# mckerrigan/shadow

Measured on AMD Instinct MI355X. Metric: source-paths/sec, higher is better.
Workload: dtype f64; 1 GPU; c4_as50k: Barabasi-Albert Internet-like topology, all-pairs latency/reliability table (BASELINE.json configs[3]); n_vertices=50000, n_edges=550000, n_edges_nonloop=500000, csr_arcs=1000000, targets=50000, table_bytes=40000000000, parallelism=one GPU

## Files before the change

### shadow_amd/csrc/engine.hip

```cpp
#include "common.hpp"

#include <array>
#include <atomic>
#include <chrono>
#include <condition_variable>
#include <functional>
#include <map>
#include <memory>
#include <mutex>
#include <sys/mman.h>

#include <thread>
#include "sssp_f64.hpp"
#include "sssp_f64d.hpp"
#include "sssp_k32.hpp"
#include "sssp_batch.hpp"
#include "path_attr.hpp"
#include "sssp_delta.hpp"
#include "direct_fw.hpp"
#include "fw.hpp"
#include "path_hops.hpp"
#include "link_loads.hpp"
#include "path_ties.hpp"
#include "ecmp_loads.hpp"
// ... 235 lines not shown
        if (rc) return rc;
        if (s.kf.h) {
            if (hipMalloc((void**)&c->d_kf_ws, s.kf.ws_stride * (size_t)s.kf.slots) != hipSuccess) return SHD_ROUTE_ENOMEM;
            c->allocs.push_back(c->d_kf_ws);
        }
    }
    c->h_ridx = std::move(s.kd.oridx);
    s.arrays([](const char*, auto& h, auto*&) { std::remove_reference_t<decltype(h)>().swap(h); });
    s.inrows.order = {}; s.inrows.src_of = {};
    c->sel = s.sel;
    c->inrows = std::move(s.inrows); c->k32 = std::move(s.k32); c->attr = s.attr;
    c->kb = std::move(s.kb); c->kd = std::move(s.kd); c->kf = std::move(s.kf);
    return SHD_ROUTE_OK;
}

DevDelta kd_args(const shd_route* c) {
    DevDelta k;
    k.n = c->n; k.nw = (c->n + 63) / 64; k.bound = c->k32.bound; k.delta = c->kd.delta;
    k.fused = c->kd.fused; k.rc = c->kd.qcap;
    k.row = c->d_row; k.orec = c->kd.d_orec; k.oridx = c->kd.d_oridx;
    k.nnz = c->nnz; k.lrow = c->kd.d_lrow; k.lrec = reinterpret_cast<const uint2*>(c->kd.d_lrec); k.nlight = c->kd.nlight;
    k.rtab = c->kd.d_rtab; k.nrtab = c->kd.nrtab; k.rone = c->kd.rone; k.walk = c->kd.walk; k.packed = c->kd.packed;
    k.vf = c->d_vf; k.self_w = c->d_self_w; k.self_r = c->d_self_r; k.dbg = c->d_dbg; k.dflags = 0;
    k.has_vf = c->vf_lossy;
#ifdef SHD_STAMPS
    if (const char* e = getenv("SHD_ROUTE_DFLAGS")) k.dflags = atoi(e);
#endif
    k.seed_drop = 0;
    if (const char* e = getenv("SHD_ROUTE_SEEDDROP")) k.seed_drop = atoi(e) & ~1;

    k.jobs = nullptr; k.drow = nullptr; k.drow_out = nullptr; k.prow = nullptr; k.rstride = 0; k.evcap = c->n;
    k.done = nullptr;
    if (const char* e = getenv("SHD_ROUTE_EVCAP")) k.evcap = std::max(0, std::min(c->n, atoi(e)));
    k.next = nullptr;
    k.stats = c->d_kd_stats;
    return k;
}

int kd_launch(shd_route* c, DevDelta k, int* next, const int32_t* d_src, int ns, const int32_t* d_tgt, int nt,
              int64_t ld, double* d_lat, double* d_rel, double* d_row_min, hipStream_t st, bool planner = false,
              char* ws = nullptr, int max_grid = 0, bool hub = false) {
    if (ns <= 0) return SHD_ROUTE_OK;
    k.next = next;
    if (!ws) ws = c->d_kd_ws;
    const int grid = std::min(ns, max_grid > 0 ? std::min(max_grid, c->kd.slots) : c->kd.slots);
    const bool big = hub && planner && c->kd.hub_block > 0;
    size_t lds = c->kd.lds;
    if (big) { k.rc = c->kd.hub_qcap; k.delta = c->kd.hub_delta; lds = c->kd.hub_lds; }
    kd_dispatch(big ? c->kd.hub_block : c->kd.block, [&](auto B) {
        constexpr int b = decltype(B)::value;
        if (planner)
            hipLaunchKernelGGL(kd_plan_rows_kernel<b>, dim3(grid), dim3(b), lds, st, k, d_src, ns, d_tgt,
                               nt, (long long)ld, d_lat, d_rel, d_row_min, c->d_err, ws, c->kd.stride);
        else
            hipLaunchKernelGGL(sssp_delta_kernel<b>, dim3(grid), dim3(b), c->kd.lds, st, k, d_src, ns, d_tgt,
                               nt, (long long)ld, d_lat, d_rel, d_row_min, c->d_err, ws, c->kd.stride);
        return 0;
    });
    return hip_check(hipGetLastError());
}

DevKB kb_args(const shd_route* c, int ns) {
    DevKB kb;
    kb.n = c->n; kb.nnz = c->nnz; kb.nseg = c->kb.nseg; kb.nhub = c->kb.nhub; kb.npart = c->kb.npart;
    kb.bound = c->k32.bound; kb.arc = c->kb.fused ? c->kb.d_farc : c->kb.d_arc; kb.row_in = c->inrows.d_irow;
    kb.seg = c->kb.d_seg; kb.hub = c->kb.d_hub;
// ... 1000 lines not shown
```

### shadow_amd/csrc/sssp_delta.hpp

```cpp
#pragma once
#include "common.hpp"

namespace shd {

constexpr int KD_P = 8;
static_assert(KD_P == 8, "owner markers are read as one u64 per lane");
constexpr int KD_TAIL = 4;
constexpr int KD_W = 8;
constexpr int KD_IMP = 192;
constexpr uint32_t KD_NONE = 0xFFFFFFFFu;
constexpr uint32_t KD_SRC_MARK = 0xFFFFFFFEu;

#define KD_GLOBAL __attribute__((address_space(1)))

#ifndef KD_NSEEDS
#define KD_NSEEDS 3
#endif
constexpr int KD_SEEDS = KD_NSEEDS;
#ifndef KD_NTLOAD
#define KD_NTLOAD 1
#endif
#ifndef KD_JUMPS
#define KD_JUMPS 1
#endif
struct __attribute__((aligned(64))) KDJob {
    int row;
    int s;
    int store;
    int nseed;
    int seed[KD_SEEDS];
    int u[KD_SEEDS];
    int wr[KD_SEEDS];
    int rec[KD_SEEDS];
};
static_assert(sizeof(KDJob) == 64, "one 64-byte job record");
constexpr uint32_t KD_EVTAG = 0xFFFF0000u;
typedef unsigned short kd_us2 __attribute__((ext_vector_type(2)));
typedef double kd_d2 __attribute__((ext_vector_type(2)));
typedef unsigned kd_u4 __attribute__((ext_vector_type(4)));
typedef unsigned kd_u2 __attribute__((ext_vector_type(2)));

struct DevDelta {
    int* next;
    const KDJob* __restrict__ jobs;
    const uint16_t* __restrict__ drow;
    uint16_t* drow_out;
    uint32_t* prow;
    long long rstride;
    int evcap;
    int* done;
    int n, nw;
    int nlight;
    int nnz;
    int bound;
    int delta;
    int fused;
    int rc;
    const int* __restrict__ row;
    const uint32_t* __restrict__ orec;
    const uint16_t* __restrict__ oridx;
    const int* __restrict__ lrow;
    const uint2* __restrict__ lrec;
    const double* __restrict__ rtab;
    int nrtab;
    int rone;
    int walk;
    int packed;
    const double* __restrict__ vf;
    const double* __restrict__ self_w;
    const double* __restrict__ self_r;
    int has_vf;
    int dflags;
    int seed_drop;
    unsigned long long* dbg;
    unsigned long long* stats;
};

constexpr int KD_NACC = 40;
#ifdef SHD_STAMPS
#define KD_ACCP (sm->acc)
#define KD_OUT (!(dflags & 1))
#define KD_DFLAGS g.dflags
// ... 99 lines not shown
        L.ring = o;
        L.rrec = o + a16(2 * (size_t)rc);
        L.qcap = (int)((wbytes - 16) / 6) & ~7;
        L.qv = o;
        L.qbeg = o + a16(2 * (size_t)L.qcap);
        o += wbytes;
        L.total = o;
        L.rtabl = a16(L.rix + (size_t)n);
        return L;
    }
};
constexpr int KD_MAXD = 32;
#ifndef KD_SDIV
#define KD_SDIV 8
#endif
#ifndef KD_SMIN
#define KD_SMIN 16
#endif
#ifndef KD_WDYN
#define KD_WDYN 1
#endif
#ifndef KD_WCAP
#define KD_WCAP 2
#endif
#ifndef KD_SEEDSPIN
#define KD_SEEDSPIN 8
#endif
#ifndef KD_BWAVES
#define KD_BWAVES 8
#endif
#ifndef KD_BHELP
#define KD_BHELP 1
#endif
#ifndef KD_WQ_N
#define KD_WQ_N 2
#endif
constexpr int KD_WQ = KD_WQ_N;
constexpr int KD_ONE = 254;
constexpr int KD_NAN = 255;
constexpr int KD_RR = 512;
template <int B>
constexpr int kd_rr() { return B >= 1024 ? KD_RR : 256; }

__host__ __device__ inline size_t kd_ws_stride(int n) {
    return a16(sizeof(double) * n) + a16(sizeof(uint32_t) * (n + 8)) + a16(8 * (size_t)n) + 256 +
           a16(sizeof(uint32_t) * (n + 8));
}
__host__ __device__ inline size_t kd_ws_wpr1(int n) {
    return a16(sizeof(double) * n) + a16(sizeof(uint32_t) * (n + 8)) + a16(8 * (size_t)n) + 256;
}
__host__ __device__ inline long long kd_row_stride(int n) { return ((long long)n + 2 + 7) & ~7ll; }

__device__ inline void lds_barrier() { asm volatile("s_waitcnt lgkmcnt(0)\n\ts_barrier" ::: "memory"); }
__device__ inline void wait_stores() { asm volatile("s_waitcnt vmcnt(0)" ::: "memory"); }

__device__ inline unsigned kd_wave_min(unsigned x) {
#pragma unroll
    for (int d = 32; d >= 1; d >>= 1) x = min(x, (unsigned)__shfl_xor((int)x, d, 64));
    return x;
}

__device__ inline unsigned kd_wave_min_dpp(unsigned x) {
    int v = (int)x;
    const int inf = (int)0xFFFFFFFFu;
    v = (int)min((unsigned)v, (unsigned)__builtin_amdgcn_update_dpp(inf, v, 0x111, 0xF, 0xF, false));
    v = (int)min((unsigned)v, (unsigned)__builtin_amdgcn_update_dpp(inf, v, 0x112, 0xF, 0xF, false));
// ... 37 lines not shown
        "ds_bpermute_b32 %5, %18, %25\n\t"
        "ds_bpermute_b32 %6, %19, %24\n\t"
        "ds_bpermute_b32 %7, %19, %25\n\t"
        "ds_bpermute_b32 %8, %20, %24\n\t"
        "ds_bpermute_b32 %9, %20, %25\n\t"
        "ds_bpermute_b32 %10, %21, %24\n\t"
        "ds_bpermute_b32 %11, %21, %25\n\t"
        "ds_bpermute_b32 %12, %22, %24\n\t"
        "ds_bpermute_b32 %13, %22, %25\n\t"
        "ds_bpermute_b32 %14, %23, %24\n\t"
        "ds_bpermute_b32 %15, %23, %25\n\t"
        "s_waitcnt lgkmcnt(0)"
        : "=&v"(ob[0]), "=&v"(od[0]), "=&v"(ob[1]), "=&v"(od[1]), "=&v"(ob[2]), "=&v"(od[2]),
          "=&v"(ob[3]), "=&v"(od[3]), "=&v"(ob[4]), "=&v"(od[4]), "=&v"(ob[5]), "=&v"(od[5]),
          "=&v"(ob[6]), "=&v"(od[6]), "=&v"(ob[7]), "=&v"(od[7])
        : "v"(a[0]), "v"(a[1]), "v"(a[2]), "v"(a[3]), "v"(a[4]), "v"(a[5]), "v"(a[6]), "v"(a[7]),
          "v"(x), "v"(y));
}

__device__ inline unsigned ld16(const uint16_t* d, int v) { return d[v]; }
__device__ inline uint32_t kd_comp(const uint4& v, int k) { return k == 0 ? v.x : k == 1 ? v.y : k == 2 ? v.z : v.w; }

__device__ inline void pop4(unsigned long long* b, int k, int v[4]) {
#pragma unroll
    for (int q = 0; q < 4; q++) {
        const unsigned long long x = *b;
        v[q] = x ? (k << 6) + __ffsll((long long)x) - 1 : -1;
        *b = x & (x - 1);
    }
}

__device__ inline void kd_relax_list(const uint32_t* wimp, int cnt, int lane, unsigned long long upto,
                                     uint32_t* dist32, unsigned long long* pend, unsigned* wmin, uint16_t* ring,
                                     int* tail, int rc, unsigned T, unsigned long long* sm_acc) {
    __builtin_amdgcn_wave_barrier();
    for (int b0 = 0; b0 < cnt; b0 += 64) {
        const bool act = b0 + lane < cnt;
        const uint32_t e = act ? wimp[b0 + lane] : 0u;
        const unsigned v = e & 0xFFFFu, nd = e >> 16, sh = (v & 1u) << 4;
        bool won = false;
        if (act) {
            uint32_t old = dist32[v >> 1];
            for (;;) {
                if (nd >= ((old >> sh) & 0xFFFFu)) break;
                const uint32_t got = atomicCAS(&dist32[v >> 1], old, (old & ~(0xFFFFu << sh)) | (nd << sh));
                if (got == old) { won = true; break; }
                old = got;
            }
        }
        const bool push = won && nd < T;
        if (won && nd >= T) { atomicOr(&pend[v >> 6], 1ull << (v & 63)); atomicMin(&wmin[v >> 6], nd); }
        const unsigned long long pm = __ballot(push);
        if (pm) {
            const int ctot = __popcll(pm);
            int qb = 0;
            if (lane == 0) qb = atomicAdd(tail, ctot);
            qb = __builtin_amdgcn_readfirstlane(qb);
            const int qk = max(0, min(ctot, rc - qb));
            const int rk = __popcll(pm & (upto >> 1));
            if (push && rk < qk) { ring[qb + rk] = (uint16_t)v; atomicAnd(&pend[v >> 6], ~(1ull << (v & 63))); }
            if (push && rk >= qk) { atomicOr(&pend[v >> 6], 1ull << (v & 63)); atomicMin(&wmin[v >> 6], nd); }
#ifdef SHD_STAMPS
            if (lane == 0 && ctot > qk) atomicAdd(&sm_acc[14], (unsigned long long)(ctot - qk));
#endif
        }
    }
    __builtin_amdgcn_wave_barrier();
}


#define SEED_VIEW()                                                                                   \
    const int nseed = __builtin_amdgcn_readfirstlane(sm->job.nseed);                                   \
    int su[KD_SEEDS], sslot[KD_SEEDS];                                                                 \
    unsigned wsu[KD_SEEDS], rsu[KD_SEEDS];                                                             \
    const uint16_t* sdrow[KD_SEEDS];                                                                   \
    const uint32_t* sprow[KD_SEEDS];                                                                   \
    _Pragma("unroll") for (int q_ = 0; q_ < KD_SEEDS; q_++) {                                          \
        const int sl_ = __builtin_amdgcn_readfirstlane(q_ < nseed ? sm->job.seed[q_] : 0);             \
        const unsigned wr_ = (unsigned)__builtin_amdgcn_readfirstlane(q_ < nseed ? sm->job.wr[q_] : 0); \
        su[q_] = __builtin_amdgcn_readfirstlane(q_ < nseed ? sm->job.u[q_] : -1);                      \
        sslot[q_] = sl_; wsu[q_] = wr_ & 0xFFFFu;                                                      \
        rsu[q_] = (unsigned)__builtin_amdgcn_readfirstlane(q_ < nseed ? sm->job.rec[q_] : 0);          \
        sdrow[q_] = g.drow + (size_t)sl_ * g.rstride;                                                  \
        sprow[q_] = g.prow + (size_t)sl_ * g.rstride;                                                  \
    }                                                                                                  \
    (void)sslot; (void)rsu; (void)sprow; (void)su

__device__ inline int kd_next_source(int* ctr, int* slot, int tid, bool all_queued = false) {
    if (tid == 0) *slot = (all_queued ? 0 : (int)gridDim.x) + atomicAdd(ctr, 1);
    __syncthreads();
    const int i = *slot;
    __syncthreads();
    return i;
}

template <class T>
__device__ __attribute__((always_inline)) inline T kd_uni(T x) {
    if constexpr (sizeof(T) == 8) {
        unsigned long long b;
// ... 747 lines not shown
                const int r1 = e0 + (int)(e1 >> 16);
                const unsigned dv = ld16(dist, v);
                uint32_t fr = KD_NONE;
                bool open = have && a0 < r1;
                while (__ballot(open)) {
                    const int a = a0 + sub;
                    const kd_u2 ra = __builtin_amdgcn_raw_buffer_load_b64(ars, (uint32_t)a << 3, 0, 0);
                    const kd_u2 rb = __builtin_amdgcn_raw_buffer_load_b64(ars, (uint32_t)a << 3, 64, 0);
                    const unsigned da = ld16(dist, (int)(ra.x & 0xFFFFu)), db = ld16(dist, (int)(rb.x & 0xFFFFu));
                    const bool ta = open && a < r1 && da + (ra.x >> 16) == dv;
                    const bool tb = open && a + 8 < r1 && db + (rb.x >> 16) == dv;
                    const unsigned ma = (unsigned)(__ballot(ta) >> (8 * gi)) & 0xFFu;
                    const unsigned mb = (unsigned)(__ballot(tb) >> (8 * gi)) & 0xFFu;
                    const uint32_t ca = (ra.x & 0xFFFFu) | (ra.y << 16) | (packed ? (ra.x >> 16) << 24 : 0u);
                    const uint32_t cb = (rb.x & 0xFFFFu) | (rb.y << 16) | (packed ? (rb.x >> 16) << 24 : 0u);
                    const unsigned mm = ma ? ma : mb;
                    const int from = 8 * gi + (mm ? __ffs((int)mm) - 1 : 0);
                    const uint32_t got = (uint32_t)__shfl((int)(ma ? ca : cb), from, 64);
                    if (open && mm) { fr = got; open = false; }
                    if (open) { a0 += 16; open = a0 < r1; }
                }
                if (sub == 0 && have) {
                    if (fr == KD_NONE) raise_err(err, SHD_ROUTE_EUNREACH);
                    wpr[v] = fr;
                }
            }
            KD_WACC(17);
        }
        wait_stores();
        KD_WACC(16);
    }
}

#define KD_KERNEL_PARAMS                                                                              \
    DevDelta g, const int* __restrict__ src, int ns, const int* __restrict__ tgt, int nt, long long ld,     \
        double* __restrict__ lat_out, double* __restrict__ rel_out, double* __restrict__ row_min,          \
        int* __restrict__ err, char* __restrict__ ws, size_t ws_stride
template <int B>
__device__ __attribute__((always_inline)) inline void kd_rows_body(KD_KERNEL_PARAMS) {
    extern __shared__ __attribute__((aligned(16))) char smem[];
    const int n = g.n, nw = g.nw;
    constexpr int RR = kd_rr<B>();
    const KDLayout<B> L = KDLayout<B>::make(n, g.rc, RR);
    KDSmall* sm = reinterpret_cast<KDSmall*>(smem);
    const int tid = threadIdx.x, lane = tid & 63, wid = tid >> 6;
    uint32_t* wkey = reinterpret_cast<uint32_t*>(smem + L.wkey) + wid * 64;
    uint32_t* wimp = reinterpret_cast<uint32_t*>(smem + L.wimp) + wid * KD_IMP;
    uint16_t* dist = reinterpret_cast<uint16_t*>(smem + L.dist);
    uint32_t* wmark = reinterpret_cast<uint32_t*>(smem + L.wmark) + wid * 2 * KD_P;
    unsigned long long* pend = reinterpret_cast<unsigned long long*>(smem + L.pend);
    unsigned* wmin = reinterpret_cast<unsigned*>(smem + L.wmin);
    unsigned long long* fix = reinterpret_cast<unsigned long long*>(smem + L.fix);
    uint16_t* ring = reinterpret_cast<uint16_t*>(smem + L.ring);
    uint2* rrec = reinterpret_cast<uint2*>(smem + L.rrec);
    uint16_t* qv = reinterpret_cast<uint16_t*>(smem + L.qv);
    int* qbeg = reinterpret_cast<int*>(smem + L.qbeg);
    unsigned long long* tmask = reinterpret_cast<unsigned long long*>(smem + L.tmask);
    unsigned* tpre = reinterpret_cast<unsigned*>(smem + L.tpre);
    const unsigned delta = (unsigned)g.delta;
    const int qcap = L.qcap;
    const unsigned wmask = g.packed ? 0xFFu : 0xFFFFu;
    const unsigned rmask = g.packed ? 0xFFu : 0xFFFFu;
    const __amdgpu_buffer_rsrc_t orsrc =
        __builtin_amdgcn_make_buffer_rsrc(const_cast<uint32_t*>(g.orec), (short)0, g.nnz * 4, 0x00020000);
    const int rc = g.rc;
    constexpr int NW = B / 64;
    const bool writer = wid == NW - 1;
    double* relv = reinterpret_cast<double*>(ws + (size_t)blockIdx.x * ws_stride);
    uint32_t* const wslice = reinterpret_cast<uint32_t*>(ws + (size_t)blockIdx.x * ws_stride + a16(sizeof(double) * n));
    uint2* const evl = reinterpret_cast<uint2*>(ws + (size_t)blockIdx.x * ws_stride + a16(sizeof(double) * n) +
                                                a16(sizeof(uint32_t) * (n + 8)));
#ifdef SHD_STAMPS
    if (tid < KD_NACC) sm->acc[tid] = 0;
    __syncthreads();
#endif
    const unsigned long long upto = lane == 63 ? ~0ull : ((2ull << lane) - 1ull);

    for (int k = tid; k < nw; k += B) tmask[k] = 0ull;
    if (tid == 0) sm->tsorted = 1;
    __syncthreads();
    for (int j = tid; j < nt; j += B) {
        const int t = tgt[j];
        const bool ok = t >= 0 && t < n && (j == 0 || tgt[j - 1] < t);
        if (!ok) sm->tsorted = 0;
        else atomicOr(&tmask[t >> 6], 1ull << (t & 63));
    }
    __syncthreads();
    if (wid == 0) {
        int run = 0;
        for (int k0 = 0; k0 < nw; k0 += 64) {
            const int k = k0 + lane;
            const int c = k < nw ? __popcll(tmask[k]) : 0;
            const int incl = kd_wave_incl_sum(c);
            if (k < nw) tpre[k] = (unsigned)(run + incl - c);
            run += __builtin_amdgcn_readlane(incl, 63);
        }
    }
    __syncthreads();
    const bool tsorted = __builtin_amdgcn_readfirstlane(sm->tsorted) != 0;
// ... 119 lines not shown
                uint32_t dw[2], rw[4];
#pragma unroll
                for (int h = 0; h < 4; h++) {
                    const int v = v0 + h;
                    unsigned dbest = 0xFFFFu, kbest = 0xFFFFFFFFu;
                    uint32_t rbest = KD_NONE;
#pragma unroll
                    for (int q = 0; q < KD_SEEDS; q++) {
                        const uint32_t d2 = (h < 2) ? dq[q].x : dq[q].y;
                        const unsigned d = (h & 1) ? (d2 >> 16) : (d2 & 0xFFFFu);
                        const unsigned c = q < nseed ? min(0xFFFFu, wsu[q] + d) : 0xFFFFFu;
                        const uint32_t p = kd_comp(pq[q], h);
                        const uint32_t r = v == su[q] ? rsu[q] : p;
                        const uint32_t k = __builtin_amdgcn_perm(~r, r, 0x07010002u);
                        if (c < dbest || (c == dbest && k < kbest)) { dbest = c; kbest = k; rbest = r; }
                    }
                    if (v >= n) dbest = 0xFFFFu;
                    if (v == s) rbest = KD_SRC_MARK;
                    if (h & 1) dw[h >> 1] |= dbest << 16;
                    else dw[h >> 1] = dbest;
                    rw[h] = rbest;
                }
                *reinterpret_cast<uint2*>(dist + v0) = make_uint2(dw[0], dw[1]);
                *reinterpret_cast<uint4*>(wpr + v0) = make_uint4(rw[0], rw[1], rw[2], rw[3]);
            }
            wait_stores();
        } else {
            for (int v = tid; v < (n + 2) / 2; v += B) reinterpret_cast<uint32_t*>(dist)[v] = 0xFFFFFFFFu;
        }
        for (int k = tid; k < nw; k += B) { pend[k] = 0ull; wmin[k] = 0xFFFFFFFFu; fix[k] = 0ull; }
        for (int q = tid; q < RR; q += B) rrec[q] = make_uint2(0u, 0xFFFFFFFFu);
        if (lane < 2 * KD_P) wmark[lane] = 0u;
        if (tid == 0) {
            sm->gmin[0] = sm->gmin[1] = 0xFFFFFFFFu;
            sm->rtail = sm->rdone = 0;
            sm->nev = 0; sm->evovf = 0;
            if constexpr (B >= 1024) {
                sm->rmin = kInfBits;
                sm->latblk = 0;
            }
            wpr_of()[s] = KD_SRC_MARK;
        }
        lds_barrier();
        KD_ACC(29);
        KD_STAMP(0);
        if (tid == 0) {
            dist[s] = 0;
            pend[s >> 6] = 1ull << (s & 63);
            wmin[s >> 6] = 0;
        }
        lds_barrier();

        unsigned T = delta;
        int par = 0;
        const int ncomp = NW - 1;
        int wnev = 0;
        KD_MARK();
        for (;;) {
            KD_COUNT(5, tid == 0 ? 1 : 0);
            {
                unsigned m0 = 0xFFFFFFFFu;
                for (int k = tid; k < nw; k += B) m0 = min(m0, wmin[k]);
                const unsigned wm = kd_wave_min_dpp(m0);
                if (lane == 0 && wm != 0xFFFFFFFFu) atomicMin(&sm->gmin[par], wm);
            }
            for (int q = tid; q < rc; q += B) ring[q] = 0xFFFFu;
            if (tid == 0) { sm->gmin[par ^ 1] = 0xFFFFFFFFu; sm->head = sm->tail = 0; sm->busy = 0; sm->nexit = 0; }
            lds_barrier();
            const unsigned m = sm->gmin[par];
            if (m == 0xFFFFFFFFu) break;
            if (m >= T) T = (m / delta + 1) * delta;
            KD_ACC(11);
            for (int k0 = 0; k0 < nw; k0 += B) {
                const int k = k0 + tid;
                unsigned long long bits = 0ull, take = 0ull;
                unsigned rest = 0xFFFFFFFFu;
                const bool act = k < nw && wmin[k] < T;
                if (act) {
                    bits = pend[k];
                    unsigned long long b = bits;
                    while (b) {
                        int v4[4];
                        pop4(&b, k, v4);
                        unsigned d4[4];
#pragma unroll
                        for (int q = 0; q < 4; q++) d4[q] = ld16(dist, v4[q] >= 0 ? v4[q] : n);
#pragma unroll
                        for (int q = 0; q < 4; q++) {
                            if (v4[q] < 0) continue;
                            if (d4[q] < T) take |= 1ull << (v4[q] & 63);
                            else rest = min(rest, d4[q]);
                        }
                    }
                }
                const int cnt = __popcll(take);
                int incl = kd_wave_incl_sum(cnt);
                int base = 0;
                if (lane == 63 && incl) base = atomicAdd(&sm->tail, incl);
                base = __builtin_amdgcn_readlane(base, 63);
                int pos = base + incl - cnt;
                if (act) {
                    unsigned long long b = take;
                    while (b) {
                        const int bi = __ffsll((long long)b) - 1;
                        b &= b - 1;
                        const int u = (k << 6) + bi;
                        if (pos < rc) ring[pos] = (uint16_t)u;
                        else {
                            take &= ~(1ull << bi);
                            rest = min(rest, (unsigned)dist[u]);
#ifdef SHD_STAMPS
                            atomicAdd(&sm->acc[15], 1ull);
#endif
                        }
                        pos++;
                    }
                    pend[k] = bits & ~take;
                    wmin[k] = rest;
                }
            }
            lds_barrier();
            if (tid == 0) sm->tail = min(sm->tail, rc);
            lds_barrier();
            KD_ACC(8);
            if (!writer) {
                auto push_rec = [&](unsigned long long m, bool mine, uint32_t x, uint32_t y) __attribute__((always_inline)) {
                    const int nr = __popcll(m);
                    int rb = 0;
                    if (lane == 0) {
                        rb = atomicAdd(&sm->rtail, nr);
                        int w8 = 0;
                        for (; rb + nr - __hip_atomic_load(&sm->rdone, __ATOMIC_RELAXED, __HIP_MEMORY_SCOPE_WORKGROUP) > RR
                               && w8 < (1 << 22); w8++)
                            __builtin_amdgcn_s_sleep(1);
                        if (w8 >= (1 << 22)) raise_err(err, SHD_ROUTE_EDEVICE);
                        if (w8 && g.stats) atomicMax(&g.stats[0], (unsigned long long)w8);
                    }
                    rb = __builtin_amdgcn_readfirstlane(rb);
                    if (mine) {
                        const int slot = (rb + __popcll(m & (upto >> 1))) & (RR - 1);
                        *reinterpret_cast<volatile unsigned long long*>(&rrec[slot]) =
                            (unsigned long long)x | ((unsigned long long)y << 32);
                    }
                };
                int spins = 0;
                for (;;) {
                    int h = 0, nn = 0;
                    if (lane == 0) {
                        if (min(__hip_atomic_load(&sm->tail, __ATOMIC_RELAXED, __HIP_MEMORY_SCOPE_WORKGROUP), rc) >
                            __hip_atomic_load(&sm->head, __ATOMIC_RELAXED, __HIP_MEMORY_SCOPE_WORKGROUP)) {
                            atomicAdd(&sm->busy, 1);
                            h = __hip_atomic_load(&sm->head, __ATOMIC_RELAXED, __HIP_MEMORY_SCOPE_WORKGROUP);
                            const int t = min(__hip_atomic_load(&sm->tail, __ATOMIC_RELAXED, __HIP_MEMORY_SCOPE_WORKGROUP), rc);
                            nn = min(64, t - h);
                            if (KD_SDIV > 0 && B >= 1024) nn = min(nn, max(KD_SMIN, (t - h + KD_SDIV - 1) / max(KD_SDIV, 1)));
                            if (nn > 0 && atomicCAS(&sm->head, h, h + nn) != h) nn = 0;
// ... 102 lines not shown
                    auto process = [&](const Win& W, const int b0) __attribute__((always_inline)) {
                        const int lb = b0 + lane;
                        unsigned dvs[KD_P];
#pragma unroll
                        for (int p = 0; p < KD_P; p++) dvs[p] = ld16(dist, (int)(W.rx[p] & 0xFFFFu));
                        auto step = [&](const int p, auto full) __attribute__((always_inline)) {
                            const unsigned v = W.rx[p] & 0xFFFFu, w = (W.rx[p] >> 16) & wmask;
                            const unsigned odu = W.odo[p] & 0xFFFFu;
                            const unsigned dv = dvs[p], nd = odu + w;
                            bool valid = true;
                            if constexpr (!decltype(full)::value) valid = lb + 64 * p < total;
                            const bool imp = valid && nd < dv;
                            const unsigned long long im = __ballot(imp);
                            if (imp) {
                                const unsigned r = __builtin_amdgcn_mbcnt_hi((unsigned)(im >> 32),
                                                   __builtin_amdgcn_mbcnt_lo((unsigned)im, (unsigned)nimp));
                                wimp[r] = v | (nd << 16);
                            }
                            nimp += __popcll(im);
                            if (g.fused && valid && dv + w == odu)
                                atomicMin(&wkey[W.odo[p] >> 16], __builtin_amdgcn_perm(~W.rx[p], W.rx[p], 0x06010003u));
                            if (seeded) {
                                const bool tie = valid && nd == dv;
                                const unsigned long long tm = __ballot(tie);
                                if (tm) {
                                    const int pv = __shfl(u, (int)(W.odo[p] >> 16), 64);
                                    push_rec(tm, tie, (uint32_t)pv | ((W.rx[p] >> 24) << 16) | (w << 24), v | KD_EVTAG);
                                }
                            }
                        };
                        static_assert(KD_IMP >= 192, "two steps between flush checks");
                        auto flush = [&]() __attribute__((always_inline)) {
                            kd_relax_list(wimp, nimp, lane, upto, reinterpret_cast<uint32_t*>(dist), pend, wmin, ring,
                                          &sm->tail, rc, T, KD_ACCP);
                            nimp = 0;
                        };
                        if (b0 + 64 * KD_P <= total) {
#pragma unroll
                            for (int p = 0; p < KD_P; p += 2) {
                                step(p, std::true_type{});
                                step(p + 1, std::true_type{});
                                if (nimp > KD_IMP - 128) flush();
                            }
                        } else {
                            const int nstep = (total - b0 + 63) >> 6;
#pragma unroll
                            for (int p = 0; p < KD_P; p += 2) {
                                if (p >= nstep) break;
                                step(p, std::false_type{});
                                if (p + 1 < nstep) step(p + 1, std::false_type{});
                                if (nimp > KD_IMP - 128) flush();
                            }
                        }
                    };
                    issue(wa, 0);
                    for (int b0 = 0; b0 < total;) {
                        issue(wb, b0 + 64 * KD_P);
                        process(wa, b0);
                        b0 += 64 * KD_P;
                        if (b0 >= total) break;
                        issue(wa, b0 + 64 * KD_P);
                        process(wb, b0);
                        b0 += 64 * KD_P;
                    }
                    if (nimp) kd_relax_list(wimp, nimp, lane, upto, reinterpret_cast<uint32_t*>(dist), pend, wmin, ring, &sm->tail, rc, T, KD_ACCP);
#ifdef SHD_STAMPS
                    if (tid == 0) { const unsigned long long t_ = __builtin_amdgcn_s_memtime(); sm->acc[23] += t_ - ks0; ks0 = t_; sm->acc[25] += (total + 64 * KD_P - 1) / (64 * KD_P); }
#endif
                    KD_COUNT(7, total);
                    KD_COUNT(6, nn);
                    KD_COUNT(20, 1);
                    __builtin_amdgcn_wave_barrier();
                    const bool hasrec = act && u != s;
                    uint32_t prec = KD_NONE;
                    if (g.fused && hasrec) {
                        const uint32_t kk = deg0 > 0 ? wkey[crank] : ~0u;
                        if (kk != ~0u && (0xFFu - (kk >> 24)) >= delta)
                            prec = ((kk >> 8) & 0xFFFFu) | ((kk & 0xFFu) << 16) | ((0xFFu - (kk >> 24)) << 24);
                    }
                    const unsigned long long rm = __ballot(hasrec);
                    if (rm) push_rec(rm, hasrec, prec, (uint32_t)u | (du0 << 16));
                    if (lane == 0) atomicSub(&sm->busy, 1);
#ifdef SHD_STAMPS
                    if (tid == 0) { const unsigned long long t_ = __builtin_amdgcn_s_memtime(); sm->acc[24] += t_ - ks0; sm->acc[26] += 1; }
#endif
                }
                if (lane == 0) atomicAdd(&sm->nexit, 1);
            } else {
                uint32_t* const wpr = wpr_of();
                int rd = __hip_atomic_load(&sm->rdone, __ATOMIC_RELAXED, __HIP_MEMORY_SCOPE_WORKGROUP);
                int spins = 0;
                for (;;) {
                    const int rt = __hip_atomic_load(&sm->rtail, __ATOMIC_RELAXED, __HIP_MEMORY_SCOPE_WORKGROUP);
                    if (rt > rd) {
                        const int k = min(min(4 * 64, RR - 64), rt - rd);
                        int uu[4], ev[4];
                        uint32_t xx[4];
#pragma unroll
// ... 37 lines not shown
                            }
                        }
                        rd += k;
                        __builtin_amdgcn_wave_barrier();
                        if (lane == 0) __hip_atomic_store(&sm->rdone, rd, __ATOMIC_RELAXED, __HIP_MEMORY_SCOPE_WORKGROUP);
                        spins = 0;
                        continue;
                    }
                    if (__hip_atomic_load(&sm->nexit, __ATOMIC_RELAXED, __HIP_MEMORY_SCOPE_WORKGROUP) == ncomp &&
                        __hip_atomic_load(&sm->rtail, __ATOMIC_RELAXED, __HIP_MEMORY_SCOPE_WORKGROUP) == rd) {
                        if (lane == 0) sm->nev = wnev;
                        break;
                    }
                    if (++spins > (1 << 22)) { if (lane == 0) raise_err(err, SHD_ROUTE_EDEVICE); break; }
                    __builtin_amdgcn_s_sleep(1);
                }
            }
            par ^= 1;
            lds_barrier();
            KD_ACC(10);
        }
        wait_stores();
        lds_barrier();
        if (seeded) {
            KD_MARK();
            const int nev = sm->nev;
            if (nev > g.evcap) {
                lds_barrier();
                if (tid == 0) sm->job.nseed = 0;
                lds_barrier();
                goto kd_restart;
            }
            uint32_t* const wpr = wpr_of();
            SEED_VIEW();
            auto d0 = [&](int v) __attribute__((always_inline)) {
                unsigned x = 0xFFFFu;
#pragma unroll
                for (int q = 0; q < KD_SEEDS; q++)
                    if (q < nseed) x = min(x, min(0xFFFFu, wsu[q] + (unsigned)sdrow[q][v]));
                return x;
            };
            KD_ACC(27);
            uint32_t* key = reinterpret_cast<uint32_t*>(relv);
            auto event = [&](int e, int& v, uint32_t& ke) __attribute__((always_inline)) {
                const uint2 r = evl[e];
                v = (int)r.y;
                const int p = (int)(r.x & 0xFFFFu);
                const unsigned w = r.x >> 24, dv = ld16(dist, v);
                if (dv != d0(v) || ld16(dist, p) + w != dv) { v = -1; return; }
                ke = ((0xFFu - w) << 24) | ((uint32_t)p << 8) | ((r.x >> 16) & 0xFFu);
            };
            for (int e = tid; e < nev; e += B) {
                int v; uint32_t ke = 0;
                event(e, v, ke);
                if (v >= 0) {
                    const uint32_t b = wpr[v];
                    const unsigned pb = b & 0xFFFFu, wb = ld16(dist, v) - ld16(dist, (int)pb);
                    key[v] = ((0xFFu - wb) << 24) | (pb << 8) | ((b >> 16) & 0xFFu);
                }
            }
            wait_stores();
            lds_barrier();
            for (int e = tid; e < nev; e += B) {
                int v; uint32_t ke = 0;
                event(e, v, ke);
                if (v >= 0) atomicMin(&key[v], ke);
            }
            wait_stores();
            lds_barrier();
            for (int e = tid; e < nev; e += B) {
                int v; uint32_t ke = 0;
                event(e, v, ke);
                if (v >= 0) {
                    const uint32_t k = __hip_atomic_load(&key[v], __ATOMIC_RELAXED, __HIP_MEMORY_SCOPE_AGENT);
                    wpr[v] = ((k >> 8) & 0xFFFFu) | ((k & 0xFFu) << 16) | ((0xFFu - (k >> 24)) << 24);
                }
            }
            wait_stores();
            lds_barrier();
            KD_ACC(28);
        }
        KD_STAMP(1);
        KD_MARK();

        const int last_arc = g.nlight > 0 ? g.nlight - 1 : 0;
        uint32_t* const wpr = wpr_of();
        if constexpr (B >= 1024) {
        static_assert(KD_BWAVES >= 1 && KD_BWAVES < NW, "B waves and store waves");
        constexpr int NSW = NW - KD_BWAVES;
        const int store = __builtin_amdgcn_readfirstlane(sm->job.store);
        KD_WDECL(wid == 0 || wid == KD_BWAVES);
        if (wid < KD_BWAVES) {
            kd_fixup<B>(s, (KD_GLOBAL uint32_t*)wpr);
            KD_WMARK();
            if (KD_BHELP && wid > 0 && i >= 0) kd_lat_row<B>(i, s, sw_s);
        } else {
            if (store >= 0) {
                uint16_t* dr = g.drow_out + (size_t)store * g.rstride;
                for (int v0 = 8 * (tid - 64 * KD_BWAVES); v0 <= n; v0 += 8 * 64 * NSW)
                    *reinterpret_cast<uint4*>(dr + v0) = *reinterpret_cast<const uint4*>(dist + v0);
                wait_stores();
            }
            KD_WACC(37);
            if (i >= 0) kd_lat_row<B>(i, s, sw_s);
            KD_WACC(38);
        }
        lds_barrier();
        if (wid == 0) KD_WACC(39);
        if (store >= 0 && tid == 0) {
            __builtin_amdgcn_fence(__ATOMIC_RELEASE, "agent");
            asm volatile("s_waitcnt vmcnt(0)" ::: "memory");
            __hip_atomic_store(&g.done[store], 1, __ATOMIC_RELAXED, __HIP_MEMORY_SCOPE_AGENT);
// ... 145 lines not shown
```

Before: 1.245 million source-paths/s.

## Track next bucket minimum during relaxation and hash-merge seed events in LDS

Two changes to the delta-stepping SSSP kernel. For blocks of at least KD_ACCMIN_B threads, the minimum distance for the next bucket is now accumulated while relaxing and compacting, instead of re-scanning all wmin words each round. The first round seeds the ring directly with the source, and the barrier that clamped the tail is removed. Seed-event fixup moves from three passes over the event list with global-memory atomics into a noinline kd_events routine. That routine filters events once and reduces them through a chunked LDS hash table before writing wpr, at the cost of LDS probing and possible table overflow errors.

```diff
diff --git a/shadow_amd/csrc/engine.hip b/shadow_amd/csrc/engine.hip
--- a/shadow_amd/csrc/engine.hip
+++ b/shadow_amd/csrc/engine.hip
@@ -291,6 +291,8 @@
     k.jobs = nullptr; k.drow = nullptr; k.drow_out = nullptr; k.prow = nullptr; k.rstride = 0; k.evcap = c->n;
     k.done = nullptr;
     if (const char* e = getenv("SHD_ROUTE_EVCAP")) k.evcap = std::max(0, std::min(c->n, atoi(e)));
+    k.evchunk = 0;
+    if (const char* e = getenv("SHD_ROUTE_EVCHUNK")) k.evchunk = std::max(0, atoi(e));
     k.next = nullptr;
     k.stats = c->d_kd_stats;
     return k;
diff --git a/shadow_amd/csrc/sssp_delta.hpp b/shadow_amd/csrc/sssp_delta.hpp
--- a/shadow_amd/csrc/sssp_delta.hpp
+++ b/shadow_amd/csrc/sssp_delta.hpp
@@ -48,6 +48,7 @@
     uint32_t* prow;
     long long rstride;
     int evcap;
+    int evchunk;
     int* done;
     int n, nw;
     int nlight;
@@ -213,6 +214,9 @@
 #ifndef KD_BHELP
 #define KD_BHELP 1
 #endif
+#ifndef KD_ACCMIN_B
+#define KD_ACCMIN_B 1024
+#endif
 #ifndef KD_WQ_N
 #define KD_WQ_N 2
 #endif
@@ -316,8 +320,9 @@
 
 __device__ inline void kd_relax_list(const uint32_t* wimp, int cnt, int lane, unsigned long long upto,
                                      uint32_t* dist32, unsigned long long* pend, unsigned* wmin, uint16_t* ring,
-                                     int* tail, int rc, unsigned T, unsigned long long* sm_acc) {
+                                     int* tail, unsigned* gnext, int rc, unsigned T, unsigned long long* sm_acc) {
     __builtin_amdgcn_wave_barrier();
+    unsigned gm = 0xFFFFFFFFu;
     for (int b0 = 0; b0 < cnt; b0 += 64) {
         const bool act = b0 + lane < cnt;
         const uint32_t e = act ? wimp[b0 + lane] : 0u;
@@ -333,7 +338,8 @@
             }
         }
         const bool push = won && nd < T;
-        if (won && nd >= T) { atomicOr(&pend[v >> 6], 1ull << (v & 63)); atomicMin(&wmin[v >> 6], nd); }
+        bool keep = won && nd >= T;
+        if (keep) { atomicOr(&pend[v >> 6], 1ull << (v & 63)); atomicMin(&wmin[v >> 6], nd); }
         const unsigned long long pm = __ballot(push);
         if (pm) {
             const int ctot = __popcll(pm);
@@ -343,12 +349,14 @@
             const int qk = max(0, min(ctot, rc - qb));
             const int rk = __popcll(pm & (upto >> 1));
             if (push && rk < qk) { ring[qb + rk] = (uint16_t)v; atomicAnd(&pend[v >> 6], ~(1ull << (v & 63))); }
-            if (push && rk >= qk) { atomicOr(&pend[v >> 6], 1ull << (v & 63)); atomicMin(&wmin[v >> 6], nd); }
+            if (push && rk >= qk) { keep = true; atomicOr(&pend[v >> 6], 1ull << (v & 63)); atomicMin(&wmin[v >> 6], nd); }
 #ifdef SHD_STAMPS
             if (lane == 0 && ctot > qk) atomicAdd(&sm_acc[14], (unsigned long long)(ctot - qk));
 #endif
         }
-    }
+        gm = min(gm, keep ? nd : 0xFFFFFFFFu);
+    }
+    if (gnext && __ballot(gm != 0xFFFFFFFFu)) { gm = kd_wave_min_dpp(gm); if (lane == 0) atomicMin(gnext, gm); }
     __builtin_amdgcn_wave_barrier();
 }
 
@@ -1162,7 +1170,86 @@
     }
 }
 
-#define KD_KERNEL_PARAMS                                                                              \
+template <int B>
+__device__ __attribute__((noinline)) void kd_events(KD_GLOBAL uint32_t* __restrict__ const wpr,
+                                                    const KD_GLOBAL kd_u2* __restrict__ const evl, const int nev,
+                                                    const int evchunk, int* __restrict__ const err) {
+    extern __shared__ __attribute__((aligned(16))) char smem[];
+    constexpr int RR = kd_rr<B>();
+    KDSmall* sm = reinterpret_cast<KDSmall*>(smem);
+    const int n = kd_uni(sm->out.n), rc = kd_uni(sm->out.rc);
+    const KDLayout<B> L = KDLayout<B>::make(n, rc, RR);
+    const int tid = threadIdx.x;
+    const uint16_t* dist = reinterpret_cast<const uint16_t*>(smem + L.dist);
+    const int nseed = kd_uni(sm->job.nseed);
+    const KD_GLOBAL uint16_t* const drow = (const KD_GLOBAL uint16_t*)kd_uni(sm->drow);
+    const long long rstride = kd_uni(sm->rstride);
+    const KD_GLOBAL uint16_t* sdrow[KD_SEEDS];
+    unsigned wsu[KD_SEEDS];
+#pragma unroll
+    for (int q = 0; q < KD_SEEDS; q++) {
+        sdrow[q] = drow + (size_t)kd_uni(q < nseed ? sm->job.seed[q] : 0) * rstride;
+        wsu[q] = (unsigned)kd_uni(q < nseed ? sm->job.wr[q] : 0) & 0xFFFFu;
+    }
+    uint32_t* const tv = reinterpret_cast<uint32_t*>(smem + L.work);
+    const size_t wbytes = a16(2 * (size_t)rc) + 8 * (size_t)RR;
+    const int hmax = 31 - __clz((int)(wbytes >> 3));
+    int chunk = 1 << (hmax - 1);
+    if (evchunk > 0) chunk = min(chunk, evchunk);
+    const int hb = max(1, min(hmax, 32 - __clz(2 * min(nev, chunk) - 1)));
+    const int H = 1 << hb;
+    uint32_t* const tk = tv + H;
+#ifdef SHD_STAMPS
+    if (tid == 0) sm->acc[34] += (unsigned long long)nev;
+#endif
+    for (int c0 = 0; c0 < nev; c0 += chunk) {
+        const int c1 = min(nev, c0 + chunk);
+        for (int t = tid; t < H; t += B) { tv[t] = 0xFFFFFFFFu; tk[t] = 0xFFFFFFFFu; }
+        lds_barrier();
+        for (int e = c0 + tid; e < c1; e += B) {
+            const kd_u2 r = evl[e];
+            const int v = (int)r.y;
+            const int p = (int)(r.x & 0xFFFFu);
+            const unsigned w = r.x >> 24, dv = ld16(dist, v);
+            const uint32_t b = __hip_atomic_load(&wpr[v], __ATOMIC_RELAXED, __HIP_MEMORY_SCOPE_AGENT);
+            unsigned d0 = 0xFFFFu;
+#pragma unroll
+            for (int q = 0; q < KD_SEEDS; q++)
+                if (q < nseed) d0 = min(d0, min(0xFFFFu, wsu[q] + (unsigned)sdrow[q][v]));
+            if (dv != d0 || ld16(dist, p) + w != dv) continue;
+            const uint32_t ke = ((0xFFu - w) << 24) | ((uint32_t)p << 8) | ((r.x >> 16) & 0xFFu);
+            const unsigned pb = b & 0xFFFFu, wb = dv - ld16(dist, (int)pb);
+            const uint32_t kb = ((0xFFu - wb) << 24) | (pb << 8) | ((b >> 16) & 0xFFu);
+#ifdef SHD_STAMPS
+            atomicAdd(&sm->acc[35], 1ull);
+#endif
+            if (ke >= kb) continue;
+            unsigned h = ((unsigned)v * 0x9E3779B1u) >> (32 - hb);
+            int pr = 0;
+            for (; pr < H; pr++) {
+                const uint32_t old = atomicCAS(&tv[h], 0xFFFFFFFFu, (uint32_t)v);
+                if (old == 0xFFFFFFFFu || old == (uint32_t)v) { atomicMin(&tk[h], ke); break; }
+                h = (h + 1) & (unsigned)(H - 1);
+            }
+            if (pr >= H) raise_err(err, SHD_ROUTE_EDEVICE);
+        }
+        lds_barrier();
+        for (int t = tid; t < H; t += B) {
+            const uint32_t v = tv[t];
+            if (v != 0xFFFFFFFFu) {
+                const uint32_t k = tk[t];
+                wpr[v] = ((k >> 8) & 0xFFFFu) | ((k & 0xFFu) << 16) | ((0xFFu - (k >> 24)) << 24);
+#ifdef SHD_STAMPS
+                atomicAdd(&sm->acc[30], 1ull);
+#endif
+            }
+        }
+        wait_stores();
+        lds_barrier();
+    }
+}
+
+#define KD_KERNEL_PARAMS                                                                         \
     DevDelta g, const int* __restrict__ src, int ns, const int* __restrict__ tgt, int nt, long long ld,     \
         double* __restrict__ lat_out, double* __restrict__ rel_out, double* __restrict__ row_min,          \
         int* __restrict__ err, char* __restrict__ ws, size_t ws_stride
@@ -1195,6 +1282,7 @@
         __builtin_amdgcn_make_buffer_rsrc(const_cast<uint32_t*>(g.orec), (short)0, g.nnz * 4, 0x00020000);
     const int rc = g.rc;
     constexpr int NW = B / 64;
+    constexpr bool accmin = B >= KD_ACCMIN_B;
     const bool writer = wid == NW - 1;
     double* relv = reinterpret_cast<double*>(ws + (size_t)blockIdx.x * ws_stride);
     uint32_t* const wslice = reinterpret_cast<uint32_t*>(ws + (size_t)blockIdx.x * ws_stride + a16(sizeof(double) * n));
@@ -1380,7 +1468,8 @@
         for (int q = tid; q < RR; q += B) rrec[q] = make_uint2(0u, 0xFFFFFFFFu);
         if (lane < 2 * KD_P) wmark[lane] = 0u;
         if (tid == 0) {
-            sm->gmin[0] = sm->gmin[1] = 0xFFFFFFFFu;
+            sm->gmin[0] = accmin ? 0u : 0xFFFFFFFFu;
+            sm->gmin[1] = 0xFFFFFFFFu;
             sm->rtail = sm->rdone = 0;
             sm->nev = 0; sm->evovf = 0;
             if constexpr (B >= 1024) {
@@ -1394,8 +1483,10 @@
         KD_STAMP(0);
         if (tid == 0) {
             dist[s] = 0;
-            pend[s >> 6] = 1ull << (s & 63);
-            wmin[s >> 6] = 0;
+            if constexpr (!accmin) {
+                pend[s >> 6] = 1ull << (s & 63);
+                wmin[s >> 6] = 0;
+            }
         }
         lds_barrier();
 
@@ -1403,27 +1494,35 @@
         int par = 0;
         const int ncomp = NW - 1;
         int wnev = 0;
+        bool round0 = accmin;
         KD_MARK();
         for (;;) {
             KD_COUNT(5, tid == 0 ? 1 : 0);
-            {
+            if constexpr (!accmin) {
                 unsigned m0 = 0xFFFFFFFFu;
                 for (int k = tid; k < nw; k += B) m0 = min(m0, wmin[k]);
                 const unsigned wm = kd_wave_min_dpp(m0);
                 if (lane == 0 && wm != 0xFFFFFFFFu) atomicMin(&sm->gmin[par], wm);
             }
             for (int q = tid; q < rc; q += B) ring[q] = 0xFFFFu;
-            if (tid == 0) { sm->gmin[par ^ 1] = 0xFFFFFFFFu; sm->head = sm->tail = 0; sm->busy = 0; sm->nexit = 0; }
+            if (tid == 0) {
+                sm->gmin[par ^ 1] = 0xFFFFFFFFu; sm->head = sm->tail = 0; sm->busy = 0; sm->nexit = 0;
+                if (round0) { ring[0] = (uint16_t)s; sm->tail = 1; }
+            }
             lds_barrier();
             const unsigned m = sm->gmin[par];
             if (m == 0xFFFFFFFFu) break;
             if (m >= T) T = (m / delta + 1) * delta;
             KD_ACC(11);
+            unsigned gnext = 0xFFFFFFFFu;
+            if (!round0) {
             for (int k0 = 0; k0 < nw; k0 += B) {
                 const int k = k0 + tid;
                 unsigned long long bits = 0ull, take = 0ull;
                 unsigned rest = 0xFFFFFFFFu;
-                const bool act = k < nw && wmin[k] < T;
+                const unsigned wk = k < nw ? wmin[k] : 0xFFFFFFFFu;
+                const bool act = wk < T;
+                if (!act) gnext = min(gnext, wk);
                 if (act) {
                     bits = pend[k];
                     unsigned long long b = bits;
@@ -1465,11 +1564,16 @@
                     }
                     pend[k] = bits & ~take;
                     wmin[k] = rest;
-                }
+                    gnext = min(gnext, rest);
+                }
+            }
+            if constexpr (accmin) {
+                const unsigned wm = kd_wave_min_dpp(gnext);
+                if (lane == 0 && wm != 0xFFFFFFFFu) atomicMin(&sm->gmin[par ^ 1], wm);
             }
             lds_barrier();
-            if (tid == 0) sm->tail = min(sm->tail, rc);
-            lds_barrier();
+            }
+            round0 = false;
             KD_ACC(8);
             if (!writer) {
                 auto push_rec = [&](unsigned long long m, bool mine, uint32_t x, uint32_t y) __attribute__((always_inline)) {
@@ -1638,7 +1742,7 @@
                         static_assert(KD_IMP >= 192, "two steps between flush checks");
                         auto flush = [&]() __attribute__((always_inline)) {
                             kd_relax_list(wimp, nimp, lane, upto, reinterpret_cast<uint32_t*>(dist), pend, wmin, ring,
-                                          &sm->tail, rc, T, KD_ACCP);
+                                          &sm->tail, accmin ? &sm->gmin[par ^ 1] : nullptr, rc, T, KD_ACCP);
                             nimp = 0;
                         };
                         if (b0 + 64 * KD_P <= total) {
@@ -1669,7 +1773,7 @@
                         process(wb, b0);
                         b0 += 64 * KD_P;
                     }
-                    if (nimp) kd_relax_list(wimp, nimp, lane, upto, reinterpret_cast<uint32_t*>(dist), pend, wmin, ring, &sm->tail, rc, T, KD_ACCP);
+                    if (nimp) kd_relax_list(wimp, nimp, lane, upto, reinterpret_cast<uint32_t*>(dist), pend, wmin, ring, &sm->tail, accmin ? &sm->gmin[par ^ 1] : nullptr, rc, T, KD_ACCP);
 #ifdef SHD_STAMPS
                     if (tid == 0) { const unsigned long long t_ = __builtin_amdgcn_s_memtime(); sm->acc[23] += t_ - ks0; ks0 = t_; sm->acc[25] += (total + 64 * KD_P - 1) / (64 * KD_P); }
 #endif
@@ -1773,52 +1877,8 @@
                 goto kd_restart;
             }
             uint32_t* const wpr = wpr_of();
-            SEED_VIEW();
-            auto d0 = [&](int v) __attribute__((always_inline)) {
-                unsigned x = 0xFFFFu;
-#pragma unroll
-                for (int q = 0; q < KD_SEEDS; q++)
-                    if (q < nseed) x = min(x, min(0xFFFFu, wsu[q] + (unsigned)sdrow[q][v]));
-                return x;
-            };
             KD_ACC(27);
-            uint32_t* key = reinterpret_cast<uint32_t*>(relv);
-            auto event = [&](int e, int& v, uint32_t& ke) __attribute__((always_inline)) {
-                const uint2 r = evl[e];
-                v = (int)r.y;
-                const int p = (int)(r.x & 0xFFFFu);
-                const unsigned w = r.x >> 24, dv = ld16(dist, v);
-                if (dv != d0(v) || ld16(dist, p) + w != dv) { v = -1; return; }
-                ke = ((0xFFu - w) << 24) | ((uint32_t)p << 8) | ((r.x >> 16) & 0xFFu);
-            };
-            for (int e = tid; e < nev; e += B) {
-                int v; uint32_t ke = 0;
-                event(e, v, ke);
-                if (v >= 0) {
-                    const uint32_t b = wpr[v];
-                    const unsigned pb = b & 0xFFFFu, wb = ld16(dist, v) - ld16(dist, (int)pb);
-                    key[v] = ((0xFFu - wb) << 24) | (pb << 8) | ((b >> 16) & 0xFFu);
-                }
-            }
-            wait_stores();
-            lds_barrier();
-            for (int e = tid; e < nev; e += B) {
-                int v; uint32_t ke = 0;
-                event(e, v, ke);
-                if (v >= 0) atomicMin(&key[v], ke);
-            }
-            wait_stores();
-            lds_barrier();
-            for (int e = tid; e < nev; e += B) {
-                int v; uint32_t ke = 0;
-                event(e, v, ke);
-                if (v >= 0) {
-                    const uint32_t k = __hip_atomic_load(&key[v], __ATOMIC_RELAXED, __HIP_MEMORY_SCOPE_AGENT);
-                    wpr[v] = ((k >> 8) & 0xFFFFu) | ((k & 0xFFu) << 16) | ((0xFFu - (k >> 24)) << 24);
-                }
-            }
-            wait_stores();
-            lds_barrier();
+            kd_events<B>((KD_GLOBAL uint32_t*)wpr, (const KD_GLOBAL kd_u2*)evl, nev, g.evchunk, err);
             KD_ACC(28);
         }
         KD_STAMP(1);
```

Result: faster. 1.263 million source-paths/s (median of 6 runs) (+1.4%).
